# lifunudt/CORB-SLAM

Measured on AMD Instinct MI355X. Metric: stereo frames/sec ORB extract+match, higher is better.
Workload: dtype u8; 1 GPU; configs[1]: ORB extract+match, synthetic 1241x376 stereo stream, 2000 feat/frame, 8 levels x1.2, FAST 20/7; warmup_frames_per_gpu=2560, batches_in_flight=1, distinct_frames=64, parallelism=1 client per GPU, replicas (no collective), inputs=resident in HBM

## Files before the change

### corb-slam_amd/csrc/orb_kernels.hip

```cpp
#include "corb_internal.h"
#include "lane_exchange.h"
#include <atomic>
#include <cstring>
#include <cstdlib>
#include "brief_pattern.h"

#define WAVE 64

struct CorbDescribeTab { uint4 patb[64]; };
__device__ CorbDescribeTab g_dsc_tab;


#define RS_ROWS 8
__global__ __launch_bounds__(256) void orb_resize_kernel(const CorbOrbParams p, int level)
{
    const CorbLevel& D = p.lv[level];
    const CorbLevel& S = p.lv[level - 1];
    const int img = p.img_base + blockIdx.z;
    const int x4 = (blockIdx.x * 64 + threadIdx.x) * 4;
    const int yb = (blockIdx.y * 4 + threadIdx.y) * RS_ROWS;
    if (x4 >= D.w || yb >= D.h) return;
    const short* tab = p.resize_tab + D.resize_tab_off;
    const short* xofs = tab, * xa0 = tab + D.w, * xa1 = tab + 2 * D.w;
    const short* ys0 = tab + 3 * D.w, * ys1 = ys0 + D.h, * yb0 = ys1 + D.h, * yb1 = yb0 + D.h;
    const uint8_t* src = p.pyr + (size_t)img * p.arena_per_image + S.plane_off;
    uint8_t* dstp = p.pyr + (size_t)img * p.arena_per_image + D.plane_off;
    int sx[4], sx1[4], a0[4], a1[4];
    int nvalid = 0;
#pragma unroll
    for (int k = 0; k < 4; k++) {
        const int x = min(x4 + k, D.w - 1);
        sx[k] = xofs[x]; sx1[k] = min(sx[k] + 1, S.w - 1); a0[k] = xa0[x]; a1[k] = xa1[x];
        nvalid += (x4 + k < D.w) ? 1 : 0;
    }
    const int yend = min(yb + RS_ROWS, D.h);
#pragma unroll 2
    for (int y = yb; y < yend; y++) {
        const uint8_t* S0 = src + (size_t)ys0[y] * S.pitch;
        const uint8_t* S1 = src + (size_t)ys1[y] * S.pitch;
        const int b0 = yb0[y], b1 = yb1[y];
        uint32_t packed = 0;
#pragma unroll
        for (int k = 0; k < 4; k++) {
            const int d0 = __mul24(S0[sx[k]], a0[k]) + __mul24(S0[sx1[k]], a1[k]);
            const int d1 = __mul24(S1[sx[k]], a0[k]) + __mul24(S1[sx1[k]], a1[k]);
            const uint32_t v = (uint32_t)((((__mul24(b0, d0 >> 4)) >> 16) + ((__mul24(b1, d1 >> 4)) >> 16) + 2) >> 2) & 0xFFu;
            packed |= v << (8 * k);
        }
        uint8_t* dst = dstp + (size_t)y * D.pitch + x4;
        if (nvalid == 4) *reinterpret_cast<uint32_t*>(dst) = packed;
        else for (int k = 0; k < nvalid; k++) dst[k] = (uint8_t)(packed >> (8 * k));
    }
}

__device__ __forceinline__ uint32_t mul24u(uint32_t a, uint32_t b) { uint32_t d; asm("v_mul_u32_u24 %0, %1, %2" : "=v"(d) : "v"(a), "v"(b)); return d; }
__device__ __forceinline__ uint32_t mad24u(uint32_t a, uint32_t b, uint32_t c) { uint32_t d; asm("v_mad_u32_u24 %0, %1, %2, %3" : "=v"(d) : "v"(a), "v"(b), "v"(c)); return d; }
template <int B> __device__ __forceinline__ uint32_t mul24_byte(uint32_t packed, uint32_t b)
{
    uint32_t d;
    if constexpr (B == 0) asm("v_mul_u32_u24_sdwa %0, %1, %2 dst_sel:DWORD dst_unused:UNUSED_PAD src0_sel:BYTE_0 src1_sel:DWORD" : "=v"(d) : "v"(packed), "v"(b));
    if constexpr (B == 1) asm("v_mul_u32_u24_sdwa %0, %1, %2 dst_sel:DWORD dst_unused:UNUSED_PAD src0_sel:BYTE_1 src1_sel:DWORD" : "=v"(d) : "v"(packed), "v"(b));
    if constexpr (B == 2) asm("v_mul_u32_u24_sdwa %0, %1, %2 dst_sel:DWORD dst_unused:UNUSED_PAD src0_sel:BYTE_2 src1_sel:DWORD" : "=v"(d) : "v"(packed), "v"(b));
    if constexpr (B == 3) asm("v_mul_u32_u24_sdwa %0, %1, %2 dst_sel:DWORD dst_unused:UNUSED_PAD src0_sel:BYTE_3 src1_sel:DWORD" : "=v"(d) : "v"(packed), "v"(b));
    return d;
}
__device__ __forceinline__ uint32_t mul24_hiword(uint32_t a, uint32_t b)
{ uint32_t d; asm("v_mul_u32_u24_sdwa %0, %1, %2 dst_sel:DWORD dst_unused:UNUSED_PAD src0_sel:WORD_1 src1_sel:DWORD" : "=v"(d) : "v"(a), "v"(b)); return d; }
__device__ __forceinline__ uint32_t add_hiwords(uint32_t a, uint32_t b)
{ uint32_t d; asm("v_add_u32_sdwa %0, %1, %2 dst_sel:DWORD dst_unused:UNUSED_PAD src0_sel:WORD_1 src1_sel:WORD_1" : "=v"(d) : "v"(a), "v"(b)); return d; }
template <int B> __device__ __forceinline__ void shr_into_byte(uint32_t& packed, uint32_t sh, uint32_t x)
{
    if constexpr (B == 0) asm("v_lshrrev_b32_sdwa %0, %1, %2 dst_sel:BYTE_0 dst_unused:UNUSED_PRESERVE src0_sel:DWORD src1_sel:DWORD" : "+v"(packed) : "v"(sh), "v"(x));
    if constexpr (B == 1) asm("v_lshrrev_b32_sdwa %0, %1, %2 dst_sel:BYTE_1 dst_unused:UNUSED_PRESERVE src0_sel:DWORD src1_sel:DWORD" : "+v"(packed) : "v"(sh), "v"(x));
    if constexpr (B == 2) asm("v_lshrrev_b32_sdwa %0, %1, %2 dst_sel:BYTE_2 dst_unused:UNUSED_PRESERVE src0_sel:DWORD src1_sel:DWORD" : "+v"(packed) : "v"(sh), "v"(x));
    if constexpr (B == 3) asm("v_lshrrev_b32_sdwa %0, %1, %2 dst_sel:BYTE_3 dst_unused:UNUSED_PRESERVE src0_sel:DWORD src1_sel:DWORD" : "+v"(packed) : "v"(sh), "v"(x));
}
__device__ __forceinline__ int pick_byte(uint32_t w0, uint32_t w1, uint32_t w2, int o)
{
    const uint32_t a = o < 4 ? w0 : (o < 8 ? w1 : w2);
    return (int)((a >> ((o & 3) * 8)) & 255u);
}

template <int K> __device__ __forceinline__ void pyr_px(uint32_t& packed, uint32_t P0, uint32_t P1, uint32_t Q0, uint32_t Q1,
                                                         uint32_t A0, uint32_t A1, uint32_t b0, uint32_t b1, uint32_t two)
{
    const uint32_t d0 = mul24_byte<K>(P0, A0) + mul24_byte<K>(P1, A1);
    const uint32_t d1 = mul24_byte<K>(Q0, A0) + mul24_byte<K>(Q1, A1);
    const uint32_t m0 = mul24_hiword(d0, b0), m1 = mul24_hiword(d1, b1);
    shr_into_byte<K>(packed, two, add_hiwords(m0, m1) + 2u);
}

#define PYR_T 256
__global__ __launch_bounds__(PYR_T, 8) void orb_pyramid_kernel(const CorbOrbParams p)
{
    const int strip = blockIdx.x / p.pyr_ctiles, ctile = blockIdx.x - strip * p.pyr_ctiles, img = p.img_base + blockIdx.y;
    uint8_t* base = p.pyr + (size_t)img * p.arena_per_image;
    const uint32_t two = 2u;
    for (int level = 1; level < p.nlevels; level++) {
        const CorbLevel& D = p.lv[level];
        const CorbLevel& S = p.lv[level - 1];
        const int2* xrec = p.resize_rec + D.resize_rec_off;
        const int2* yrec = xrec + ((D.w + 3) & ~3);
        const uint8_t* src = base + S.plane_off;
        uint8_t* dstp = base + D.plane_off;
        const int r0 = p.pyr_r0[strip][level], r1 = p.pyr_r1[strip][level];
        const int gfirst = p.pyr_g0[ctile][level], ngroups = p.pyr_g1[ctile][level];
        for (int gbase = gfirst; gbase < ngroups; gbase += PYR_T) {
            const int XW = min(ngroups - gbase, PYR_T), RY = PYR_T / XW;
            const int ty = (int)threadIdx.x / XW, tx = (int)threadIdx.x - ty * XW;
            if (ty >= RY) continue;
            const int x4 = (gbase + tx) * 4;
            int sx[4], sx1[4];
            uint32_t A0[4], A1[4];
            int nvalid = 0;
            const int4 xr01 = *reinterpret_cast<const int4*>(xrec + x4), xr23 = *reinterpret_cast<const int4*>(xrec + x4 + 2);
            const int xs[4] = {xr01.x, xr01.z, xr23.x, xr23.z}, xa[4] = {xr01.y, xr01.w, xr23.y, xr23.w};
#pragma unroll
            for (int k = 0; k < 4; k++) {
                sx[k] = xs[k]; sx1[k] = min(sx[k] + 1, S.w - 1);
                A0[k] = (uint32_t)(xa[k] & 0xFFFF) << 12; A1[k] = (uint32_t)(xa[k] >> 16) << 12;
                nvalid += (x4 + k < D.w) ? 1 : 0;
            }
            const int bx = sx[0] & ~3;
            const bool wide = (sx1[3] - bx) < 12;
            uint32_t s1a = 0, s2a = 0, s1b = 0, s2b = 0;
#pragma unroll
            for (int k = 0; k < 4; k++) {
                const int oa = sx[k] - bx, ob = sx1[k] - bx;
                s1a |= (uint32_t)(oa < 8 ? oa : 0x0c) << (8 * k); s2a |= (uint32_t)(oa < 8 ? k : oa - 4) << (8 * k);
                s1b |= (uint32_t)(ob < 8 ? ob : 0x0c) << (8 * k); s2b |= (uint32_t)(ob < 8 ? k : ob - 4) << (8 * k);
            }
            const bool patch_a = __any(wide && sx[3] - bx >= 8), patch_b = __any(wide && sx1[3] - bx >= 8);
            if (wide) {
                auto fetch = [&](const int2 yr, uint32_t (&w)[6], uint32_t& bb) {
                    const uint32_t* q0 = reinterpret_cast<const uint32_t*>(src + (uint32_t)(__mul24(yr.x & 0xFFFF, S.pitch) + bx));
                    const uint32_t* q1 = reinterpret_cast<const uint32_t*>(src + (uint32_t)(__mul24(yr.x >> 16, S.pitch) + bx));
                    w[0] = q0[0]; w[1] = q0[1]; w[2] = q0[2]; w[3] = q1[0]; w[4] = q1[1]; w[5] = q1[2];
                    bb = (uint32_t)yr.y;
                };
                auto emit = [&](int y, const uint32_t (&w)[6], uint32_t bb) {
                    const uint32_t b0 = bb & 0xFFFFu, b1 = bb >> 16;
                    uint32_t P0 = __builtin_amdgcn_perm(w[1], w[0], s1a), P1 = __builtin_amdgcn_perm(w[1], w[0], s1b);
                    uint32_t Q0 = __builtin_amdgcn_perm(w[4], w[3], s1a), Q1 = __builtin_amdgcn_perm(w[4], w[3], s1b);
                    if (patch_a) { P0 = __builtin_amdgcn_perm(w[2], P0, s2a); Q0 = __builtin_amdgcn_perm(w[5], Q0, s2a); }
                    if (patch_b) { P1 = __builtin_amdgcn_perm(w[2], P1, s2b); Q1 = __builtin_amdgcn_perm(w[5], Q1, s2b); }
                    uint32_t packed = 0;
                    pyr_px<0>(packed, P0, P1, Q0, Q1, A0[0], A1[0], b0, b1, two);
                    pyr_px<1>(packed, P0, P1, Q0, Q1, A0[1], A1[1], b0, b1, two);
                    pyr_px<2>(packed, P0, P1, Q0, Q1, A0[2], A1[2], b0, b1, two);
                    pyr_px<3>(packed, P0, P1, Q0, Q1, A0[3], A1[3], b0, b1, two);
                    uint8_t* dst = dstp + (uint32_t)(__mul24(y, D.pitch) + x4);
                    if (nvalid == 4) *reinterpret_cast<uint32_t*>(dst) = packed;
                    else for (int k = 0; k < nvalid; k++) dst[k] = (uint8_t)(packed >> (8 * k));
                };
                int y = r0 + ty;
                const int ylast = max(r1 - 1, 0);
                int2 ya = yrec[min(y, ylast)], yb = yrec[min(y + RY, ylast)];
                int2 yc = yrec[min(y + 2 * RY, ylast)], yd = yrec[min(y + 3 * RY, ylast)];
#pragma unroll 1
                for (; y + 3 * RY < r1; y += 4 * RY) {
                    uint32_t wa[6], wb[6], wc[6], wd[6], ba, bb, bc, bd;
                    fetch(ya, wa, ba); fetch(yb, wb, bb); fetch(yc, wc, bc); fetch(yd, wd, bd);
                    const int2 na = yrec[min(y + 4 * RY, ylast)], nb = yrec[min(y + 5 * RY, ylast)], nc = yrec[min(y + 6 * RY, ylast)], nd = yrec[min(y + 7 * RY, ylast)];
                    emit(y, wa, ba); emit(y + RY, wb, bb); emit(y + 2 * RY, wc, bc); emit(y + 3 * RY, wd, bd);
                    ya = na; yb = nb; yc = nc; yd = nd;
                }
                if (y + RY < r1) {
                    uint32_t wa[6], wb[6], ba, bb;
                    fetch(ya, wa, ba); fetch(yb, wb, bb);
                    emit(y, wa, ba); emit(y + RY, wb, bb);
                    y += 2 * RY; ya = yc; yb = yd;
                }
                if (y < r1) { uint32_t wa[6], ba; fetch(ya, wa, ba); emit(y, wa, ba); }
            } else {
#pragma unroll 1
                for (int y = r0 + ty; y < r1; y += RY) {
                    const int2 yr = yrec[y];
                    const uint8_t* S0 = src + (uint32_t)__mul24(yr.x & 0xFFFF, S.pitch);
                    const uint8_t* S1 = src + (uint32_t)__mul24(yr.x >> 16, S.pitch);
                    const uint32_t b0 = yr.y & 0xFFFF, b1 = (uint32_t)yr.y >> 16;
                    uint32_t packed = 0;
#pragma unroll
                    for (int k = 0; k < 4; k++) {
                        const uint32_t d0 = mad24u(S0[sx[k]], A0[k] >> 12, mul24u(S0[sx1[k]], A1[k] >> 12));
                        const uint32_t d1 = mad24u(S1[sx[k]], A0[k] >> 12, mul24u(S1[sx1[k]], A1[k] >> 12));
                        const uint32_t v = (((mul24u(b0, d0 >> 4) >> 16) + (mul24u(b1, d1 >> 4) >> 16) + 2u) >> 2) & 0xFFu;
                        packed |= v << (8 * k);
                    }
                    uint8_t* dst = dstp + (uint32_t)(__mul24(y, D.pitch) + x4);
                    if (nvalid == 4) *reinterpret_cast<uint32_t*>(dst) = packed;
                    else for (int k = 0; k < nvalid; k++) dst[k] = (uint8_t)(packed >> (8 * k));
                }
            }
        }
        __threadfence_block();
        __syncthreads();
    }
}


__device__ __forceinline__ uint32_t pk_min3(uint32_t a, uint32_t b, uint32_t c)
{ uint32_t d; asm("v_pk_minimum3_f16 %0, %1, %2, %3" : "=v"(d) : "v"(a), "v"(b), "v"(c)); return d; }
__device__ __forceinline__ uint32_t pk_max3(uint32_t a, uint32_t b, uint32_t c)
{ uint32_t d; asm("v_pk_maximum3_f16 %0, %1, %2, %3" : "=v"(d) : "v"(a), "v"(b), "v"(c)); return d; }
template <int K> __device__ __forceinline__ uint32_t pk_pair(const uint32_t (&w)[3])
{
    static_assert(K >= 0 && K <= 10, "window");
    if constexpr (K <= 6) return __builtin_amdgcn_perm(w[1], w[0], 0x0c000c00u | (uint32_t)K | ((uint32_t)(K + 1) << 16));
    else return __builtin_amdgcn_perm(w[2], w[1], 0x0c000c00u | (uint32_t)(K - 4) | ((uint32_t)(K - 3) << 16));
}
typedef short corb_short2 __attribute__((ext_vector_type(2)));

template <bool BRIGHT> __device__ __forceinline__ uint32_t fast_arc_chain(const uint32_t (&v)[16])
{
    auto in3 = [](uint32_t a, uint32_t b, uint32_t c) { return BRIGHT ? pk_min3(a, b, c) : pk_max3(a, b, c); };
    auto out3 = [](uint32_t a, uint32_t b, uint32_t c) { return BRIGHT ? pk_max3(a, b, c) : pk_min3(a, b, c); };
    uint32_t w3[16], w9[16], r5[5];
#pragma unroll
    for (int i = 0; i < 16; i++) w3[i] = in3(v[i], v[(i + 1) & 15], v[(i + 2) & 15]);
#pragma unroll
    for (int i = 0; i < 16; i++) w9[i] = in3(w3[i], w3[(i + 3) & 15], w3[(i + 6) & 15]);
#pragma unroll
    for (int i = 0; i < 5; i++) r5[i] = out3(w9[3 * i], w9[3 * i + 1], w9[3 * i + 2]);
    return out3(out3(r5[0], r5[1], r5[2]), out3(r5[3], r5[4], w9[15]), r5[0]);
}

template <int J> __device__ __forceinline__ uint32_t fast_pair_score(const uint32_t (&R)[7][3], uint32_t th2, uint32_t kb, uint32_t kd)
{
    constexpr int C = 4 + 2 * J;
    uint32_t v[16];
    v[0] = pk_pair<C>(R[6]);      v[1] = pk_pair<C + 1>(R[6]);  v[2] = pk_pair<C + 2>(R[5]);  v[3] = pk_pair<C + 3>(R[4]);
    v[4] = pk_pair<C + 3>(R[3]);  v[5] = pk_pair<C + 3>(R[2]);  v[6] = pk_pair<C + 2>(R[1]);  v[7] = pk_pair<C + 1>(R[0]);
    v[8] = pk_pair<C>(R[0]);      v[9] = pk_pair<C - 1>(R[0]);  v[10] = pk_pair<C - 2>(R[1]); v[11] = pk_pair<C - 3>(R[2]);
    v[12] = pk_pair<C - 3>(R[3]); v[13] = pk_pair<C - 3>(R[4]); v[14] = pk_pair<C - 2>(R[5]); v[15] = pk_pair<C - 1>(R[6]);
    const uint32_t cpk = pk_pair<C>(R[3]);
    const uint32_t e0 = pk_max3(v[0], v[8], v[8]), e1 = pk_max3(v[4], v[12], v[12]), f0 = pk_min3(v[0], v[8], v[8]), f1 = pk_min3(v[4], v[12], v[12]);
    const uint32_t m = pk_min3(e0, e1, e1), n = pk_max3(f0, f1, f1);
    const uint32_t nbright = (cpk + kb) - m;
    const uint32_t dark = ((cpk + kd) - n) & 0x02000200u;
    const uint32_t donly = dark & nbright, both = dark ^ donly;
    const uint32_t xm = (donly >> 1) - (donly >> 9);
#pragma unroll
    for (int i = 0; i < 16; i++) v[i] ^= xm;
    const corb_short2 c = __builtin_bit_cast(corb_short2, cpk ^ xm) + (short)1;
    corb_short2 s = __builtin_bit_cast(corb_short2, fast_arc_chain<true>(v)) - c;
    if (__any(both != 0u)) s = __builtin_elementwise_max(s, c - (short)2 - __builtin_bit_cast(corb_short2, fast_arc_chain<false>(v)));
    const corb_short2 keep = s >= __builtin_bit_cast(corb_short2, th2);
    return __builtin_bit_cast(uint32_t, (corb_short2)(s & keep));
}

template <int J> __device__ __forceinline__ uint32_t fast_compass(const uint32_t (&R0)[3], const uint32_t (&R3)[3], const uint32_t (&R6)[3])
{
    constexpr int C = 4 + 2 * J;
    const uint32_t v0 = pk_pair<C>(R6), v4 = pk_pair<C + 3>(R3), v8 = pk_pair<C>(R0), v12 = pk_pair<C - 3>(R3), cpk = pk_pair<C>(R3);
    const uint32_t m = pk_min3(pk_max3(v0, v8, v8), pk_max3(v4, v12, v12), pk_max3(v4, v12, v12));
    const uint32_t n = pk_max3(pk_min3(v0, v8, v8), pk_min3(v4, v12, v12), pk_min3(v4, v12, v12));
    const corb_short2 c = __builtin_bit_cast(corb_short2, cpk);
    return __builtin_bit_cast(uint32_t, __builtin_elementwise_max(__builtin_bit_cast(corb_short2, m) - c, c - __builtin_bit_cast(corb_short2, n)));
}
__device__ __forceinline__ int mbcnt64(unsigned long long m) { return (int)__builtin_amdgcn_mbcnt_hi((uint32_t)(m >> 32), __builtin_amdgcn_mbcnt_lo((uint32_t)m, 0u)); }

#define FAST_LIST_CAP 512
__device__ __forceinline__ int wave_incl_scan(int v)
{
    v += __builtin_amdgcn_update_dpp(0, v, 0x111, 0xf, 0xf, true);
    v += __builtin_amdgcn_update_dpp(0, v, 0x112, 0xf, 0xf, true);
    v += __builtin_amdgcn_update_dpp(0, v, 0x114, 0xf, 0xf, true);
    v += __builtin_amdgcn_update_dpp(0, v, 0x118, 0xf, 0xf, true);
    v += __builtin_amdgcn_update_dpp(0, v, 0x142, 0xa, 0xf, true);
    v += __builtin_amdgcn_update_dpp(0, v, 0x143, 0xc, 0xf, true);
    return v;
}
template <int TP>
__global__ __launch_bounds__(64) void orb_fast_kernel(const CorbOrbParams p)
{
    constexpr int P = TP / 4;
    extern __shared__ __attribute__((aligned(16))) uint8_t fast_smem[];
    __shared__ uint16_t plist[FAST_LIST_CAP];
    uint32_t* tile = reinterpret_cast<uint32_t*>(fast_smem);
    uint32_t* sc = tile + P * p.fast_th;
    uint32_t (*rowm)[2] = reinterpret_cast<uint32_t (*)[2]>(sc + P * p.fast_th);
    const int nrowm = p.fast_th - 6;
    uint8_t* scb = reinterpret_cast<uint8_t*>(sc);
    int cell, img; corb_xcd_remap(cell, img); img += p.img_base;
    const int lane = threadIdx.x;
    uint4 rec = reinterpret_cast<const uint4*>(p.fast_cells)[cell];
    asm volatile("" : "+s"(rec.x));
    int* out_count = p.cell_count + (size_t)img * p.cells_per_image + cell;
    if (rec.y >> 31) { if (lane == 0) *out_count = 0; return; }
    const CorbLevel& L = p.lv[(rec.y >> 24) & 15u];
    const int c = cell - L.cell_base;
    const int ox = (int)(rec.y & 0xFFFu), oy = (int)((rec.y >> 12) & 0xFFFu);
    const int cw = (int)(rec.z & 0xFFu), ch = (int)((rec.z >> 8) & 0xFFu);
    const int iw = cw - 6, ih = ch - 6;
    {
        const uint32_t a = (uint32_t)ox & 3u;
        const uint8_t* src = p.pyr + (size_t)img * p.arena_per_image + rec.x;
        const int jlast = (int)(rec.w >> 20);
        const int r0 = lane / P, wc = lane - r0 * P;
        constexpr int RPI = 64 / P;
        if (r0 < RPI) {
            const int j0 = min(wc, jlast), j1 = min(wc + 1, jlast);
            for (int y = r0; y < ch; y += 4 * RPI) {
                uint32_t w0[4], w1[4];
#pragma unroll
                for (int k = 0; k < 4; k++) {
                    const uint32_t* g = reinterpret_cast<const uint32_t*>(src + (uint32_t)__mul24(min(y + k * RPI, ch - 1), L.pitch));
                    w0[k] = g[j0]; w1[k] = g[j1];
                }
#pragma unroll
                for (int k = 0; k < 4; k++)
                    if (y + k * RPI < ch) { tile[(y + k * RPI) * P + wc] = __builtin_amdgcn_alignbyte(w1[k], w0[k], a); sc[(y + k * RPI) * P + wc] = 0u; }
            }
        }
    }
    __syncthreads();
    const int rstep = (int)((rec.z >> 16) & 0xFFu), ng = (int)(rec.z >> 24);
    const int r = (int)(((uint32_t)lane * (rec.w & 0xFFFFFu)) >> 16), g = lane - r * ng;
    const bool active = r < rstep;
    const int nvalid = min(4, iw - 4 * g);
    const uint32_t smask0 = nvalid >= 2 ? 0x80008000u : nvalid == 1 ? 0x00008000u : 0u, smask1 = nvalid >= 4 ? 0x80008000u : nvalid == 3 ? 0x00008000u : 0u;
    unsigned long long mine = 0;
    for (int pass = 0; pass < 2; pass++) {
        const int th = pass == 0 ? p.ini_th : p.min_th;
        const uint32_t th2 = (uint32_t)th * 0x00010001u;
        const uint32_t kb = th2 + 0x02000200u, kd = 0x02000200u - th2 - 0x00010001u;
        if (lane < nrowm) { rowm[lane][0] = 0u; rowm[lane][1] = 0u; }
        int y0 = 3, nbatch = 0, base = 0, nscore = 0;
        while (y0 < ch - 3) {
            nbatch++;
            base = 0;
            for (; y0 < ch - 3 && base + 128 <= FAST_LIST_CAP; y0 += rstep) {
                const int y = y0 + r;
                bool hit0 = false, hit1 = false;
                if (active && y < ch - 3) {
                    const uint32_t* t = tile + y * P + g;
                    uint32_t R0[3], R3[3], R6[3];
#pragma unroll
                    for (int k = 0; k < 3; k++) { R0[k] = t[-3 * P + k]; R3[k] = t[k]; R6[k] = t[3 * P + k]; }
                    const uint32_t d0 = __builtin_bit_cast(uint32_t, (corb_short2)(__builtin_bit_cast(corb_short2, th2) - __builtin_bit_cast(corb_short2, fast_compass<0>(R0, R3, R6))));
                    const uint32_t d1 = __builtin_bit_cast(uint32_t, (corb_short2)(__builtin_bit_cast(corb_short2, th2) - __builtin_bit_cast(corb_short2, fast_compass<1>(R0, R3, R6))));
                    hit0 = (d0 & smask0) != 0u; hit1 = (d1 & smask1) != 0u;
                }
                const unsigned long long b0 = __ballot(hit0), b1 = __ballot(hit1);
                const int n0 = __popcll(b0);
                const uint32_t ent = (uint32_t)((y << 6) | (g << 1));
                if (hit0) plist[base + mbcnt64(b0)] = (uint16_t)ent;
                if (hit1) plist[base + n0 + mbcnt64(b1)] = (uint16_t)(ent | 1u);
                base += n0 + __popcll(b1);
            }
            __syncthreads();
            nscore = 0;
            for (int i0 = 0; i0 < base; i0 += 64) {
                const int i = i0 + lane;
                bool has = false;
                uint32_t e = 0;
                if (i < base) {
                e = plist[i];
                const int y = e >> 6, ge = (e >> 1) & 31;
                const uint32_t sh = (e & 1u) * 2u;
                const uint32_t* t = tile + y * P + ge;
                uint32_t R[7][3];
#pragma unroll
                for (int dy = 0; dy < 7; dy++) {
                    const uint32_t w0 = t[(dy - 3) * P], w1 = t[(dy - 3) * P + 1], w2 = t[(dy - 3) * P + 2];
                    R[dy][0] = __builtin_amdgcn_alignbyte(w1, w0, sh); R[dy][1] = __builtin_amdgcn_alignbyte(w2, w1, sh); R[dy][2] = __builtin_amdgcn_alignbyte(0u, w2, sh);
                }
                const uint32_t s0 = fast_pair_score<0>(R, th2, kb, kd);
                const int px = 4 * ge + (int)sh;
                uint32_t v = __builtin_amdgcn_perm(0u, s0, 0x0c0c0200u);
                if (px + 1 >= iw) v &= 0xFFu;
                reinterpret_cast<uint16_t*>(scb)[(y * TP + 4 + px) >> 1] = (uint16_t)v;
                has = v != 0u;
                }
                const unsigned long long bs = __ballot(has);
                if (has) plist[nscore + mbcnt64(bs)] = (uint16_t)e;
                nscore += __popcll(bs);
            }
            __syncthreads();
        }
        auto nms_group = [&](int y, int ge) {
            const uint32_t* t = sc + y * P + ge;
            if (t[1] == 0u) return;
            uint32_t S[3][3];
#pragma unroll
            for (int dy = 0; dy < 3; dy++)
#pragma unroll
                for (int k = 0; k < 3; k++) S[dy][k] = t[(dy - 1) * P + k];
            uint32_t bits = 0;
#pragma unroll
            for (int j = 0; j < 2; j++) {
                uint32_t ctr, nb;
                if (j == 0) {
                    ctr = pk_pair<4>(S[1]);
                    nb = pk_max3(pk_max3(pk_pair<3>(S[0]), pk_pair<4>(S[0]), pk_pair<5>(S[0])),
                                 pk_max3(pk_pair<3>(S[2]), pk_pair<4>(S[2]), pk_pair<5>(S[2])),
                                 pk_max3(pk_pair<3>(S[1]), pk_pair<5>(S[1]), pk_pair<5>(S[1])));
                } else {
                    ctr = pk_pair<6>(S[1]);
                    nb = pk_max3(pk_max3(pk_pair<5>(S[0]), pk_pair<6>(S[0]), pk_pair<7>(S[0])),
                                 pk_max3(pk_pair<5>(S[2]), pk_pair<6>(S[2]), pk_pair<7>(S[2])),
                                 pk_max3(pk_pair<5>(S[1]), pk_pair<7>(S[1]), pk_pair<7>(S[1])));
                }
                const uint32_t dm = __builtin_bit_cast(uint32_t, (corb_short2)(__builtin_bit_cast(corb_short2, nb) - __builtin_bit_cast(corb_short2, ctr)));
                bits |= (((dm >> 15) & 1u) | ((dm >> 30) & 2u)) << (2 * j);
            }
            if (bits) atomicOr(&rowm[y - 3][ge >> 3], bits << (4 * (ge & 7)));
        };
        if (nbatch == 1) {
            for (int i = lane; i < nscore; i += 64) {
                const uint32_t e = plist[i];
                const int y = e >> 6, ge = (e >> 1) & 31;
                const uint32_t sh = (e & 1u) * 2u;
                const uint32_t* t = sc + y * P + ge;
                uint32_t S[3][3];
#pragma unroll
                for (int dy = 0; dy < 3; dy++) {
                    const uint32_t w0 = t[(dy - 1) * P], w1 = t[(dy - 1) * P + 1], w2 = t[(dy - 1) * P + 2];
                    S[dy][0] = __builtin_amdgcn_alignbyte(w1, w0, sh); S[dy][1] = __builtin_amdgcn_alignbyte(w2, w1, sh); S[dy][2] = 0u;
                }
                const uint32_t ctr = pk_pair<4>(S[1]);
                const uint32_t nb = pk_max3(pk_max3(pk_pair<3>(S[0]), pk_pair<4>(S[0]), pk_pair<5>(S[0])),
                                            pk_max3(pk_pair<3>(S[2]), pk_pair<4>(S[2]), pk_pair<5>(S[2])),
                                            pk_max3(pk_pair<3>(S[1]), pk_pair<5>(S[1]), pk_pair<5>(S[1])));
                const uint32_t dm = __builtin_bit_cast(uint32_t, (corb_short2)(__builtin_bit_cast(corb_short2, nb) - __builtin_bit_cast(corb_short2, ctr)));
                const uint32_t bits = ((dm >> 15) & 1u) | ((dm >> 30) & 2u);
                if (bits) atomicOr(&rowm[y - 3][ge >> 3], bits << (4 * (ge & 7) + sh));
            }
        } else if (active) {
            for (int y = 3 + r; y < ch - 3; y += rstep) nms_group(y, g);
        }
        __syncthreads();
        mine = lane < ih ? ((unsigned long long)rowm[lane][1] << 32) | rowm[lane][0] : 0ull;
        if (__any(mine != 0ull)) break;
        __syncthreads();
    }
    unsigned long long mask = mine;
    const int cnt = __popcll(mask);
    const int incl = wave_incl_scan(cnt);
    const int total = __builtin_amdgcn_readlane(incl, 63);
    uint32_t* out = p.cand + (size_t)img * p.cand_per_image + L.cand_base + (size_t)c * L.cell_cap;
    int off = incl - cnt;
    while (mask) {
        const int x = __ffsll((long long)mask) - 1;
        mask &= mask - 1;
        if (off < L.cell_cap)
            out[off] = (uint32_t)(ox + x) | ((uint32_t)(oy + lane) << 12) |
                       ((uint32_t)scb[(lane + 3) * TP + x + 4] << 24);
        off++;
    }
    if (lane == 0) { *out_count = min(total, L.cell_cap); if (total > L.cell_cap) p.status[img] = CORB_ERR_OVERFLOW; }
}

#define BL_ROWS 32
#define BL_CHUNK 8
__device__ __forceinline__ int reflect101(int v, int n) { if (v < 0) v = -v; if (v >= n) v = 2 * n - 2 - v; return min(max(v, 0), n - 1); }
#define BLW4(b0, b1, b2, b3) ((uint32_t)(b0) | ((uint32_t)(b1) << 8) | ((uint32_t)(b2) << 16) | ((uint32_t)(b3) << 24))
#define BLW2(lo, hi) ((uint32_t)(lo) | ((uint32_t)(hi) << 16))
typedef unsigned short bl_us2 __attribute__((ext_vector_type(2)));
__device__ __forceinline__ uint32_t bl_dot2(uint32_t a, uint32_t w, uint32_t c)
{ return __builtin_amdgcn_udot2(__builtin_bit_cast(bl_us2, a), __builtin_bit_cast(bl_us2, w), c, false); }
__device__ __forceinline__ uint32_t bl_sat_pk(uint32_t a) { uint32_t d; asm("v_sat_pk_u8_i16 %0, %1" : "=v"(d) : "v"(a)); return d; }

template <bool INTERIOR>
__device__ __forceinline__ void blur_strip(const uint8_t* __restrict__ src, uint8_t* __restrict__ dst, int x, int y0, int y1, int h, int pitch, int wimg)
{
    const int xl = max(x - 4, 0);
    auto load_chunk = [&](uint32_t (&W)[BL_CHUNK][3], int first_row) {
        if (__all(first_row >= 0 && first_row + BL_CHUNK <= h)) {
            const uint32_t o0 = (uint32_t)__mul24(first_row, pitch) + (uint32_t)xl;
#pragma unroll
            for (int i = 0; i < BL_CHUNK; i++) {
                const uint32_t* row = reinterpret_cast<const uint32_t*>(src + (o0 + (uint32_t)(i * pitch)));
                W[i][0] = row[0]; W[i][1] = row[1]; W[i][2] = row[2];
            }
            return;
        }
#pragma unroll
        for (int i = 0; i < BL_CHUNK; i++) {
            const uint32_t off = (uint32_t)__mul24(reflect101(first_row + i, h), pitch) + (uint32_t)xl;
// ... 778 lines not shown
```

Measured before the change: 108,600 stereo frames/s.

## Restructure pyramid resize into per-wave contiguous row runs with horizontal-pass reuse

The pyramid kernel now gives each wave a contiguous quarter of the strip's rows and lets each lane walk consecutive output rows instead of strided ones. Because adjacent output rows often share a source row, the horizontally interpolated bottom row is kept and reused as the next row's top row, so those loads and that arithmetic are skipped. y-records are read through a constant address-space pointer, and a uniform-row fast path uses scalar row indices when a wave covers a single run. This cuts redundant global loads and horizontal math, but adds divergence and complexity. Chunk widths may also leave lanes idle on narrow levels.

```diff
diff --git a/corb-slam_amd/csrc/orb_kernels.hip b/corb-slam_amd/csrc/orb_kernels.hip
--- a/corb-slam_amd/csrc/orb_kernels.hip
+++ b/corb-slam_amd/csrc/orb_kernels.hip
@@ -91,24 +91,36 @@
 }
 
 #define PYR_T 256
+typedef const uint64_t __attribute__((address_space(4)))* pyr_yrec_ptr;
+struct PyrUni { static constexpr bool value = true; };
+struct PyrLane { static constexpr bool value = false; };
+__device__ __forceinline__ int pyr_chunk_width(int rem)
+{
+    if (rem >= 64) return 64;
+    return (64 / rem) * rem * 4 >= 3 * 64 ? rem : 1 << (31 - __clz(rem));
+}
 __global__ __launch_bounds__(PYR_T, 8) void orb_pyramid_kernel(const CorbOrbParams p)
 {
     const int strip = blockIdx.x / p.pyr_ctiles, ctile = blockIdx.x - strip * p.pyr_ctiles, img = p.img_base + blockIdx.y;
     uint8_t* base = p.pyr + (size_t)img * p.arena_per_image;
     const uint32_t two = 2u;
+    const int wave = __builtin_amdgcn_readfirstlane((int)threadIdx.x >> 6), lane = (int)threadIdx.x & 63;
     for (int level = 1; level < p.nlevels; level++) {
         const CorbLevel& D = p.lv[level];
         const CorbLevel& S = p.lv[level - 1];
         const int2* xrec = p.resize_rec + D.resize_rec_off;
-        const int2* yrec = xrec + ((D.w + 3) & ~3);
+        const pyr_yrec_ptr yrec = (pyr_yrec_ptr)(uintptr_t)(xrec + ((D.w + 3) & ~3));
         const uint8_t* src = base + S.plane_off;
         uint8_t* dstp = base + D.plane_off;
         const int r0 = p.pyr_r0[strip][level], r1 = p.pyr_r1[strip][level];
-        const int gfirst = p.pyr_g0[ctile][level], ngroups = p.pyr_g1[ctile][level];
-        for (int gbase = gfirst; gbase < ngroups; gbase += PYR_T) {
-            const int XW = min(ngroups - gbase, PYR_T), RY = PYR_T / XW;
-            const int ty = (int)threadIdx.x / XW, tx = (int)threadIdx.x - ty * XW;
-            if (ty >= RY) continue;
+        const int gfirst = p.pyr_g0[ctile][level], gend = p.pyr_g1[ctile][level];
+        const int wq = (r1 - r0 + 3) >> 2, wr0 = r0 + wave * wq, wr1 = min(wr0 + wq, r1);
+        for (int gbase = gfirst, W = 0; gbase < gend && wr0 < wr1; gbase += W) {
+            W = pyr_chunk_width(gend - gbase);
+            const int R = 64 / W, len = (wr1 - wr0 + R - 1) / R;
+            const int run = lane / W, tx = lane - run * W;
+            const int y0 = wr0 + run * len, y1 = min(y0 + len, wr1);
+            if (run >= R || y0 >= y1) continue;
             const int x4 = (gbase + tx) * 4;
             int sx[4], sx1[4];
             uint32_t A0[4], A1[4];
@@ -130,52 +142,92 @@
                 s1a |= (uint32_t)(oa < 8 ? oa : 0x0c) << (8 * k); s2a |= (uint32_t)(oa < 8 ? k : oa - 4) << (8 * k);
                 s1b |= (uint32_t)(ob < 8 ? ob : 0x0c) << (8 * k); s2b |= (uint32_t)(ob < 8 ? k : ob - 4) << (8 * k);
             }
-            const bool patch_a = __any(wide && sx[3] - bx >= 8), patch_b = __any(wide && sx1[3] - bx >= 8);
             if (wide) {
-                auto fetch = [&](const int2 yr, uint32_t (&w)[6], uint32_t& bb) {
-                    const uint32_t* q0 = reinterpret_cast<const uint32_t*>(src + (uint32_t)(__mul24(yr.x & 0xFFFF, S.pitch) + bx));
-                    const uint32_t* q1 = reinterpret_cast<const uint32_t*>(src + (uint32_t)(__mul24(yr.x >> 16, S.pitch) + bx));
-                    w[0] = q0[0]; w[1] = q0[1]; w[2] = q0[2]; w[3] = q1[0]; w[4] = q1[1]; w[5] = q1[2];
-                    bb = (uint32_t)yr.y;
+                auto hpass = [&](const uint32_t (&w)[3], uint32_t (&d)[4]) {
+                    const uint32_t P0 = __builtin_amdgcn_perm(w[2], __builtin_amdgcn_perm(w[1], w[0], s1a), s2a), P1 = __builtin_amdgcn_perm(w[2], __builtin_amdgcn_perm(w[1], w[0], s1b), s2b);
+                    d[0] = mul24_byte<0>(P0, A0[0]) + mul24_byte<0>(P1, A1[0]); d[1] = mul24_byte<1>(P0, A0[1]) + mul24_byte<1>(P1, A1[1]);
+                    d[2] = mul24_byte<2>(P0, A0[2]) + mul24_byte<2>(P1, A1[2]); d[3] = mul24_byte<3>(P0, A0[3]) + mul24_byte<3>(P1, A1[3]);
                 };
-                auto emit = [&](int y, const uint32_t (&w)[6], uint32_t bb) {
-                    const uint32_t b0 = bb & 0xFFFFu, b1 = bb >> 16;
-                    uint32_t P0 = __builtin_amdgcn_perm(w[1], w[0], s1a), P1 = __builtin_amdgcn_perm(w[1], w[0], s1b);
-                    uint32_t Q0 = __builtin_amdgcn_perm(w[4], w[3], s1a), Q1 = __builtin_amdgcn_perm(w[4], w[3], s1b);
-                    if (patch_a) { P0 = __builtin_amdgcn_perm(w[2], P0, s2a); Q0 = __builtin_amdgcn_perm(w[5], Q0, s2a); }
-                    if (patch_b) { P1 = __builtin_amdgcn_perm(w[2], P1, s2b); Q1 = __builtin_amdgcn_perm(w[5], Q1, s2b); }
-                    uint32_t packed = 0;
-                    pyr_px<0>(packed, P0, P1, Q0, Q1, A0[0], A1[0], b0, b1, two);
-                    pyr_px<1>(packed, P0, P1, Q0, Q1, A0[1], A1[1], b0, b1, two);
-                    pyr_px<2>(packed, P0, P1, Q0, Q1, A0[2], A1[2], b0, b1, two);
-                    pyr_px<3>(packed, P0, P1, Q0, Q1, A0[3], A1[3], b0, b1, two);
-                    uint8_t* dst = dstp + (uint32_t)(__mul24(y, D.pitch) + x4);
-                    if (nvalid == 4) *reinterpret_cast<uint32_t*>(dst) = packed;
-                    else for (int k = 0; k < nvalid; k++) dst[k] = (uint8_t)(packed >> (8 * k));
+                auto rows = [&](auto mode) {
+                    constexpr bool UNI = decltype(mode)::value;
+                    auto uni = [](int v) { if constexpr (UNI) return __builtin_amdgcn_readfirstlane(v); else return v; };
+                    auto rec = [&](int yy) { const uint64_t v = yrec[yy]; return make_uint2((uint32_t)v, (uint32_t)(v >> 32)); };
+                    auto fresh = [](uint32_t s0, uint32_t kept) -> bool { if constexpr (UNI) return s0 != kept; else return __any(s0 != kept) != 0; };
+                    auto load_row = [&](uint32_t s, uint32_t (&w)[3]) {
+                        const uint32_t* q;
+                        if constexpr (UNI) q = reinterpret_cast<const uint32_t*>(src + s * (uint32_t)S.pitch + (uint32_t)bx);
+                        else q = reinterpret_cast<const uint32_t*>(src + (uint32_t)(__mul24((int)s, S.pitch) + bx));
+                        w[0] = q[0]; w[1] = q[1]; w[2] = q[2];
+                    };
+                    uint32_t dk[4] = {0u, 0u, 0u, 0u};
+                    uint32_t kept = 0xFFFFu;
+                    auto emit = [&](int yy, bool fr, const uint32_t (&t)[3], const uint32_t (&b)[3], uint32_t bb) {
+                        const uint32_t b0 = bb & 0xFFFFu, b1 = bb >> 16;
+                        uint32_t dt[4];
+                        if (fr) hpass(t, dt);
+                        else { dt[0] = dk[0]; dt[1] = dk[1]; dt[2] = dk[2]; dt[3] = dk[3]; }
+                        hpass(b, dk);
+                        uint32_t packed = 0;
+                        shr_into_byte<0>(packed, two, add_hiwords(mul24_hiword(dt[0], b0), mul24_hiword(dk[0], b1)) + 2u);
+                        shr_into_byte<1>(packed, two, add_hiwords(mul24_hiword(dt[1], b0), mul24_hiword(dk[1], b1)) + 2u);
+                        shr_into_byte<2>(packed, two, add_hiwords(mul24_hiword(dt[2], b0), mul24_hiword(dk[2], b1)) + 2u);
+                        shr_into_byte<3>(packed, two, add_hiwords(mul24_hiword(dt[3], b0), mul24_hiword(dk[3], b1)) + 2u);
+                        uint8_t* dst;
+                        if constexpr (UNI) dst = dstp + (uint32_t)yy * (uint32_t)D.pitch + (uint32_t)x4;
+                        else dst = dstp + (uint32_t)(__mul24(yy, D.pitch) + x4);
+                        if (nvalid == 4) *reinterpret_cast<uint32_t*>(dst) = packed;
+                        else for (int k = 0; k < nvalid; k++) dst[k] = (uint8_t)(packed >> (8 * k));
+                    };
+                    int y = uni(y0);
+                    const int yend = uni(y1), ylast = r1 - 1;
+                    uint2 ra = rec(min(y, ylast)), rb = rec(min(y + 1, ylast));
+                    if constexpr (UNI) {
+                        uint2 rc = rec(min(y + 2, ylast)), rd = rec(min(y + 3, ylast));
+#pragma unroll 1
+                        for (; y + 3 < yend; y += 4) {
+                            uint32_t ta[3], tb[3], tc[3], td[3], ba[3], bb[3], bc[3], bd[3];
+                            const bool fa = fresh(ra.x & 0xFFFFu, kept), fb = fresh(rb.x & 0xFFFFu, ra.x >> 16), fc = fresh(rc.x & 0xFFFFu, rb.x >> 16), fd = fresh(rd.x & 0xFFFFu, rc.x >> 16);
+                            if (fa) load_row(ra.x & 0xFFFFu, ta);
+                            load_row(ra.x >> 16, ba);
+                            if (fb) load_row(rb.x & 0xFFFFu, tb);
+                            load_row(rb.x >> 16, bb);
+                            if (fc) load_row(rc.x & 0xFFFFu, tc);
+                            load_row(rc.x >> 16, bc);
+                            if (fd) load_row(rd.x & 0xFFFFu, td);
+                            load_row(rd.x >> 16, bd);
+                            const uint2 na = rec(min(y + 4, ylast)), nb = rec(min(y + 5, ylast)), nc = rec(min(y + 6, ylast)), nd = rec(min(y + 7, ylast));
+                            emit(y, fa, ta, ba, ra.y); emit(y + 1, fb, tb, bb, rb.y); emit(y + 2, fc, tc, bc, rc.y); emit(y + 3, fd, td, bd, rd.y);
+                            kept = rd.x >> 16;
+                            ra = na; rb = nb; rc = nc; rd = nd;
+                        }
+                    }
+#pragma unroll 1
+                    for (; y + 1 < yend; y += 2) {
+                        uint32_t ta[3], tb[3], ba[3], bb[3];
+                        const bool fa = fresh(ra.x & 0xFFFFu, kept), fb = fresh(rb.x & 0xFFFFu, ra.x >> 16);
+                        if (fa) load_row(ra.x & 0xFFFFu, ta);
+                        load_row(ra.x >> 16, ba);
+                        if (fb) load_row(rb.x & 0xFFFFu, tb);
+                        load_row(rb.x >> 16, bb);
+                        const uint2 na = rec(min(y + 2, ylast)), nb = rec(min(y + 3, ylast));
+                        emit(y, fa, ta, ba, ra.y); emit(y + 1, fb, tb, bb, rb.y);
+                        kept = rb.x >> 16;
+                        ra = na; rb = nb;
+                    }
+                    if (y < yend) {
+                        uint32_t ta[3], ba[3];
+                        const bool fa = fresh(ra.x & 0xFFFFu, kept);
+                        if (fa) load_row(ra.x & 0xFFFFu, ta);
+                        load_row(ra.x >> 16, ba);
+                        emit(y, fa, ta, ba, ra.y);
+                    }
                 };
-                int y = r0 + ty;
-                const int ylast = max(r1 - 1, 0);
-                int2 ya = yrec[min(y, ylast)], yb = yrec[min(y + RY, ylast)];
-                int2 yc = yrec[min(y + 2 * RY, ylast)], yd = yrec[min(y + 3 * RY, ylast)];
-#pragma unroll 1
-                for (; y + 3 * RY < r1; y += 4 * RY) {
-                    uint32_t wa[6], wb[6], wc[6], wd[6], ba, bb, bc, bd;
-                    fetch(ya, wa, ba); fetch(yb, wb, bb); fetch(yc, wc, bc); fetch(yd, wd, bd);
-                    const int2 na = yrec[min(y + 4 * RY, ylast)], nb = yrec[min(y + 5 * RY, ylast)], nc = yrec[min(y + 6 * RY, ylast)], nd = yrec[min(y + 7 * RY, ylast)];
-                    emit(y, wa, ba); emit(y + RY, wb, bb); emit(y + 2 * RY, wc, bc); emit(y + 3 * RY, wd, bd);
-                    ya = na; yb = nb; yc = nc; yd = nd;
-                }
-                if (y + RY < r1) {
-                    uint32_t wa[6], wb[6], ba, bb;
-                    fetch(ya, wa, ba); fetch(yb, wb, bb);
-                    emit(y, wa, ba); emit(y + RY, wb, bb);
-                    y += 2 * RY; ya = yc; yb = yd;
-                }
-                if (y < r1) { uint32_t wa[6], ba; fetch(ya, wa, ba); emit(y, wa, ba); }
+                if (R == 1) rows(PyrUni{}); else rows(PyrLane{});
             } else {
 #pragma unroll 1
-                for (int y = r0 + ty; y < r1; y += RY) {
-                    const int2 yr = yrec[y];
+                for (int y = y0; y < y1; y++) {
+                    const uint64_t yv = yrec[y];
+                    const int2 yr = make_int2((int)(uint32_t)yv, (int)(uint32_t)(yv >> 32));
                     const uint8_t* S0 = src + (uint32_t)__mul24(yr.x & 0xFFFF, S.pitch);
                     const uint8_t* S1 = src + (uint32_t)__mul24(yr.x >> 16, S.pitch);
                     const uint32_t b0 = yr.y & 0xFFFF, b1 = (uint32_t)yr.y >> 16;
```

New measurement: 110,500 stereo frames/s (median of 6 runs). 1.02x the previous value.
